# prashantpandeygit/solvingpapers

Measured on AMD Instinct MI355X. Metric: training tokens/sec, LLaMA3-8B-shape bf16, higher is better.
Workload: dtype bf16; 1 GPU; model=llama3_8b, global_batch=4, seq_len=8192, parallelism=dp1, micro_batch=1, grad_accum=4, params=8030261248

## Files before the change

### csrc/include/attn_params.h

```cpp
#pragma once
#include "attn_common.h"

#define SPA_DBG_BRH(b, r, R, h, H) (SPA_DBG_OK(b, p.B) & SPA_DBG_OK(r, R) & SPA_DBG_OK(h, H))

namespace spa {

struct AttnParams {
  const bf16* q; const bf16* k; const bf16* v; const bf16* o; const bf16* dout;
  bf16* out; bf16* dq; bf16* dk; bf16* dv;
  float* lse; const float* lse_in; float* delta; float* dqacc;
  int B, H, Hkv, Tq, Tk;
  long sqb, sqt, sqh, skb, skt, skh, svb, svt, svh, sob, sot, soh;
  long sdob, sdot, sdoh;
  long sdqb, sdqt, sdqh, sdkb, sdkt, sdkh, sdvb, sdvt, sdvh;
  float scale;
  float scale_log2;
  int causal_off;
  int hsplit;
  float* dkacc; float* dvacc;
  unsigned seed_lo, seed_hi, drop_thr;
  float drop_scale;
  const int64_t* seed_ptr;
  long long* stamp;
  int xcd;
  bf16* dsbuf;
  long ds_kvstride;
  int ds_nqt, ds_nkt;
  int ksplit;
  float* part;
  float* mlpart;
  int part_ld;
  int vhalf;
  float* rowk;
  int rowk_ld;
};

void launch_dkdv5(AttnParams& p, bool causal, hipStream_t st);
void launch_bwd_short(AttnParams& p, bool causal, hipStream_t st);

__device__ __forceinline__ long ds_index(int qt, int kt, int g, int G, int nkt, bool causal) {
  const int qb = qt >> 1, t = qt & 1;
  const long step = causal ? (long)qb * (qb + 1) + kt : (long)qb * nkt + kt;
  return (step * G + g) * 2 + t;
}
inline long ds_kv_elems(int nq64, int nkt, int G, bool causal) {
  return 1024L * 2 * G * (causal ? (long)nq64 * (nq64 + 1) : (long)nq64 * nkt);
}
__device__ __forceinline__ int ds_slot(int s, int h, int k) { return (k >> 2) * 16 + (2 * s + h) * 4 + (k & 3); }

template <int HD, int NDT = HD / 32>
__device__ __forceinline__ void store_kv_grad(const AttnParams& p, const f32x16 (&acc)[NDT], bool is_k,
                                              int b, int hk, int key, int split, int hh, int dt0 = 0) {
  if (key >= p.Tk) return;
  if (!(SPA_DBG_BRH(b, key, p.Tk, hk, p.Hkv) & SPA_DBG_OK(split, p.hsplit))) return;
  static_assert(NDT <= HD / 32, "store_kv_grad: more tiles than the head dim");
  constexpr int DT = NDT;
  if (p.hsplit == 1) {
    bf16* dst = (is_k ? p.dk + b * p.sdkb + (long)key * p.sdkt + hk * p.sdkh
                      : p.dv + b * p.sdvb + (long)key * p.sdvt + hk * p.sdvh) + 32 * dt0;
    const float sc = is_k ? p.scale : 1.f;
#pragma unroll
    for (int dt = 0; dt < DT; ++dt)
#pragma unroll
      for (int g = 0; g < 4; ++g) {
        bf16x4 w;
#pragma unroll
        for (int i = 0; i < 4; ++i) w[i] = (bf16)(acc[dt][4 * g + i] * sc);
        *reinterpret_cast<bf16x4*>(dst + 32 * dt + 8 * g + 4 * hh) = w;
      }
  } else {
    float* dst = (is_k ? p.dkacc : p.dvacc) +
                 ((((long)split * p.B + b) * p.Tk + key) * p.Hkv + hk) * HD + 32 * dt0;
#pragma unroll
    for (int dt = 0; dt < DT; ++dt)
#pragma unroll
      for (int g = 0; g < 4; ++g) {
        f32x4 w;
#pragma unroll
        for (int i = 0; i < 4; ++i) w[i] = acc[dt][4 * g + i];
        *reinterpret_cast<f32x4*>(dst + 32 * dt + 8 * g + 4 * hh) = w;
      }
  }
// ... 5 lines not shown
```

### csrc/include/spa_common.h

```cpp
#pragma once

#include <hip/hip_runtime.h>
#include <torch/library.h>
#include <ATen/ATen.h>
#include <ATen/hip/HIPContext.h>
#include <ATen/hip/impl/HIPGuardImplMasqueradingAsCUDA.h>
#include <cstdint>

#include "spa_debug.h"

namespace spa {

typedef __bf16 bf16;
typedef __bf16 bf16x8 __attribute__((ext_vector_type(8)));
typedef __bf16 bf16x4 __attribute__((ext_vector_type(4)));
typedef __bf16 bf16x2 __attribute__((ext_vector_type(2)));
typedef float f32x16 __attribute__((ext_vector_type(16)));
typedef float f32x4 __attribute__((ext_vector_type(4)));
typedef float f32x2 __attribute__((ext_vector_type(2)));
typedef unsigned short u16x8 __attribute__((ext_vector_type(8)));

constexpr int kWave = 64;

using DeviceGuard = c10::hip::HIPGuardMasqueradingAsCUDA;
// ... 30 lines not shown
}
template <int NT>
__device__ __forceinline__ float block_max(float v, float* red) {
  v = wave_max(v);
  const int w = threadIdx.x >> 6, l = threadIdx.x & 63;
  if (NT == 64) return v;
  __syncthreads();
  if (l == 0) red[w] = v;
  __syncthreads();
  float s = -INFINITY;
#pragma unroll
  for (int i = 0; i < NT / 64; ++i) s = fmaxf(s, red[i]);
  return s;
}

__device__ __forceinline__ void load8(const bf16* p, float (&f)[8]) {
  bf16x8 v = *reinterpret_cast<const bf16x8*>(p);
#pragma unroll
  for (int i = 0; i < 8; ++i) f[i] = (float)v[i];
}
__device__ __forceinline__ void store8(bf16* p, const float (&f)[8]) {
  bf16x8 v;
#pragma unroll
  for (int i = 0; i < 8; ++i) v[i] = (bf16)f[i];
  *reinterpret_cast<bf16x8*>(p) = v;
}
__device__ __forceinline__ void load8(const float* p, float (&f)[8]) {
  f32x4 a = *reinterpret_cast<const f32x4*>(p);
  f32x4 b = *reinterpret_cast<const f32x4*>(p + 4);
#pragma unroll
// ... 30 lines not shown
```

### csrc/kernels/attention.hip

```cpp
#include "attn_common.h"
#include "attn_params.h"

SPA_DEBUG_TU("attention.hip")

namespace spa {



__device__ __forceinline__ unsigned mix32(unsigned x) {
  x ^= x >> 16; x *= 0x7feb352dU; x ^= x >> 15; x *= 0x846ca68bU; x ^= x >> 16;
  return x;
}
__device__ __forceinline__ unsigned drop_base(const AttnParams& p, int b, int h) {
  unsigned lo = p.seed_lo, hi = p.seed_hi;
  if (p.seed_ptr) {
    const uint64_t sd = (uint64_t)*p.seed_ptr;
    lo = (unsigned)(sd & 0xffffffffu);
    hi = (unsigned)(sd >> 32);
  }
  return mix32(lo ^ mix32(hi + (unsigned)(b * p.H + h) * 0x9E3779B9U));
}
__device__ __forceinline__ bool drop_keep(unsigned base, int q, int key, unsigned thr) {
  return (mix32(base + (unsigned)q * 0x85EBCA6BU + (unsigned)key * 0xC2B2AE35U) >> 8) >= thr;
}
// ... 185 lines not shown
          for (int i = 0; i < 4; ++i) w[i] = o[dt][4 * g + i];
          *reinterpret_cast<f32x4*>(dst + 32 * dt + 8 * g + 4 * hh) = w;
        }
      if (hh == 0 && blockIdx.y == 0) {
        float2 ml;
        ml.x = m;
        ml.y = l;
        reinterpret_cast<float2*>(p.mlpart)[row] = ml;
      }
    }
    return;
  }
  const float inv = l > 0.f ? 1.f / l : 0.f;
  if (q < p.Tq && SPA_DBG_BRH(b, q, p.Tq, h, p.H)) {
    bf16* op = p.out + b * p.sob + (long)q * p.sot + h * p.soh + vcol;
#pragma unroll
    for (int dt = 0; dt < DT; ++dt)
#pragma unroll
      for (int g = 0; g < 4; ++g) {
        bf16x4 w;
#pragma unroll
        for (int i = 0; i < 4; ++i) w[i] = (bf16)(o[dt][4 * g + i] * inv);
        *reinterpret_cast<bf16x4*>(op + 32 * dt + 8 * g + 4 * hh) = w;
      }
    if (hh == 0 && p.lse)
      p.lse[((long)b * p.H + h) * p.Tq + q] = (l > 0.f) ? (m + __log2f(l)) * 0.69314718055994531f : INFINITY;
  }
}

template <bool CAUSAL>
__global__ __launch_bounds__(512) void attn_fwd256p_kernel(AttnParams p) {
  constexpr int HD = 256, BN = 32, BM = 128, KS = HD / 16, DH = 4, NT = 512;
  constexpr int TI = BN * HD;
  constexpr int PS = 4 * 2 * 64 * 8;
  __shared__ __attribute__((aligned(16))) bf16 smem[4 * TI + 2 * PS];
  __shared__ __attribute__((aligned(16))) float arow[2][4][64];
  const int tid = threadIdx.x, lane = tid & 63;
  const int wave = __builtin_amdgcn_readfirstlane(tid >> 6);
// ... 1073 lines not shown
        if (jj + 1 < nsteps) asm volatile("s_waitcnt vmcnt(6)" ::: "memory");
        else asm volatile("s_waitcnt vmcnt(0)" ::: "memory");
        asm volatile("s_waitcnt lgkmcnt(0)" ::: "memory");
        __builtin_amdgcn_s_barrier();
        if (jj + 2 < nsteps) issue(jj + 2, (r + 2) % 3);
        compute(jj, smem + r * SLOT);
      }
    }
  }
  if (!uvalid) return;
#pragma unroll
  for (int t = 0; t < 2; ++t) {
    const int q = qb * 64 + 32 * t + (lane & 31);
    if (q >= p.Tq || !SPA_DBG_BRH(b, q, p.Tq, h, p.H)) continue;
    bf16* op = p.dq + b * p.sdqb + (long)q * p.sdqt + h * p.sdqh;
#pragma unroll
    for (int dt = 0; dt < DT; ++dt)
#pragma unroll
      for (int g = 0; g < 4; ++g) {
        bf16x4 wv;
#pragma unroll
        for (int i = 0; i < 4; ++i) wv[i] = (bf16)(acc[t][dt][4 * g + i] * p.scale);
        *reinterpret_cast<bf16x4*>(op + 32 * dt + 8 * g + 4 * hh) = wv;
      }
  }
}

template <int HDK, bool CAUSAL, bool NT>
__global__ __launch_bounds__(256, 2) void attn_bwd_dq_ds256_kernel(AttnParams p) {
  static_assert(HDK == 256 || HDK == 192, "dq_ds256: q/k head dim 192 or 256");
  constexpr int HD = 256, DT = HDK / 32, KIMG = 32 * HD, WSLOT = 1024, SLOT = KIMG + 4 * WSLOT, NSLOT = 3;
  __shared__ __attribute__((aligned(16))) bf16 smem[NSLOT * SLOT];
  const int tid = threadIdx.x, lane = tid & 63;
  const int wave = __builtin_amdgcn_readfirstlane(tid >> 6);
  const int hh = lane >> 5;
  const int G = p.H / p.Hkv;
  const int nqt = cdiv(p.Tq, 32);
// ... 244 lines not shown
  constexpr int TPR = HD / 8;
  const long n = (long)p.B * p.Tq * p.H * TPR;
  for (long i = blockIdx.x * 256L + threadIdx.x; i < n; i += (long)gridDim.x * 256) {
    const int t = i % TPR;
    const long row = i / TPR;
    const long h = row % p.H, q = (row / p.H) % p.Tq, b = row / ((long)p.H * p.Tq);
    float a[8];
    load8(p.dqacc + row * HD + 8 * t, a);
#pragma unroll
    for (int k = 0; k < 8; ++k) a[k] *= p.scale;
    if (SPA_DBG_BRH(b, q, p.Tq, h, p.H)) store8(p.dq + b * p.sdqb + q * p.sdqt + h * p.sdqh + 8 * t, a);
  }
}


static void check_qkv(const at::Tensor& t, const char* n) {
  TORCH_CHECK(t.is_cuda() && t.scalar_type() == at::kBFloat16, n, " must be a bf16 HIP tensor");
  TORCH_CHECK(t.dim() == 4, n, " must be [B, T, H, hd]");
  TORCH_CHECK(t.stride(3) == 1, n, " must be contiguous in hd");
  TORCH_CHECK(((uintptr_t)t.data_ptr() % 16) == 0 && t.stride(1) % 8 == 0 && t.stride(2) % 8 == 0 &&
                  t.stride(0) % 8 == 0,
              n, ": rows must be 16-byte aligned");
}

template <int HDK, int HDV> constexpr int fwd_waves() {
  return (HDK <= 192 && HDV <= 192) || (HDK == 256 && HDV == 128) ? 8 : 4;
}
template <int HDK, int HDV> constexpr int dq_waves() { return (HDK <= 128 && HDV <= 128) ? 8 : 4; }

#define HDKV_SWITCH(HK, HV, ...)                                                                   \
// ... 26 lines not shown
  p.seed_hi = (unsigned)(((uint64_t)seed >> 32) & 0xffffffffu);
  p.drop_thr = (unsigned)std::llround(dropout_p * 16777216.0);
  p.drop_scale = (float)(1.0 / (1.0 - dropout_p));
}

static int attn_ksplit(long blocks, int ntk) {
  const char* e = getenv("SPA_ATTN_KSPLIT");
  if (e) return std::max(1, std::min(atoi(e), std::max(1, ntk)));
  int ks = 1;
  while (blocks * ks < 512 && ks < 8 && ntk / (2 * ks) >= 4) ks *= 2;
  return ks;
}

std::vector<at::Tensor> attn_fwd(const at::Tensor& q, const at::Tensor& k, const at::Tensor& v, double scale,
                                 bool causal, double dropout_p, int64_t seed,
                                 const c10::optional<at::Tensor>& seed_t) {
  check_qkv(q, "q"); check_qkv(k, "k"); check_qkv(v, "v");
  const int B = q.size(0), Tq = q.size(1), H = q.size(2), HDK = q.size(3), HDV = v.size(3);
  const int Tk = k.size(1), Hkv = k.size(2);
  TORCH_CHECK(k.size(0) == B && v.size(0) == B && v.size(1) == Tk && v.size(2) == Hkv && k.size(3) == HDK,
              "attn: shape mismatch");
  TORCH_CHECK(H % Hkv == 0, "attn: H must be a multiple of Hkv");
  const bool drop = dropout_p > 0.0;
  TORCH_CHECK(!drop || HDK == HDV, "attn: dropout needs equal q/k and v head dims");
  DeviceGuard g(q.device());
  auto out = at::empty({B, Tq, H, HDV}, q.options());
  auto lse = at::empty({B, H, Tq}, q.options().dtype(at::kFloat));
  AttnParams p{};
  p.q = (const bf16*)q.data_ptr(); p.k = (const bf16*)k.data_ptr(); p.v = (const bf16*)v.data_ptr();
  p.out = (bf16*)out.data_ptr(); p.lse = lse.data_ptr<float>();
  p.B = B; p.H = H; p.Hkv = Hkv; p.Tq = Tq; p.Tk = Tk;
  fill_strides(p, q, k, v);
  fill_dropout(p, dropout_p, seed, seed_t);
  p.sob = out.stride(0); p.sot = out.stride(1); p.soh = out.stride(2);
  p.scale = (float)scale; p.scale_log2 = (float)(scale * 1.4426950408889634);
  p.causal_off = Tk - Tq;
  p.hsplit = 1;
  p.ksplit = 1;
  p.xcd = xcd_order(B, Hkv);
  if (B * Tq * H == 0) return {out, lse};
  auto st = stream();
  const char* f2e = getenv("SPA_ATTN_FWD256");
  const bool pshare = !(f2e && atoi(f2e) == 0) && HDK == 256 && HDV == 256 && !drop;
  const char* sve = getenv("SPA_ATTN_SPLITV");
  const bool splitv = !pshare && !(sve && atoi(sve) == 0) && HDK == 256 && HDV == 256 && !drop;
  const int nw = splitv || pshare ? 8 : (HDK <= 192 && HDV <= 192) || (HDK == 256 && HDV == 128) ? 8 : 4;
  const int blocks = cdiv(Tq, pshare ? 128 : 32 * nw) * H * B * (splitv ? 2 : 1);
  const int ntk = cdiv(Tk, (HDK >= 256 || HDV >= 256) ? 32 : 64);
  p.ksplit = attn_ksplit(blocks, ntk);
  at::Tensor part;
  if (p.ksplit > 1) {
    const long rows = (long)B * H * Tq;
    part = at::empty({(long)p.ksplit * rows * (HDV + 2)}, q.options().dtype(at::kFloat));
    p.part = part.data_ptr<float>();
    p.part_ld = HDV;
    p.mlpart = p.part + (long)p.ksplit * rows * HDV;
  }
  const int gx = blocks / (splitv ? 2 : 1) * p.ksplit;
  if (pshare) {
    if (causal) attn_fwd256p_kernel<true><<<gx, 512, 0, st>>>(p);
    else attn_fwd256p_kernel<false><<<gx, 512, 0, st>>>(p);
  } else if (splitv) {
    p.vhalf = 128;
    if (causal) attn_fwd_kernel<256, 128, 8, true, false><<<dim3(gx, 2), 512, 0, st>>>(p);
    else attn_fwd_kernel<256, 128, 8, false, false><<<dim3(gx, 2), 512, 0, st>>>(p);
  } else {
    HDKV_SWITCH(HDK, HDV, {
      constexpr int NW = fwd_waves<HDK_, HDV_>();
      constexpr bool SQ = HDK_ == HDV_;
      if (drop) {
        if constexpr (SQ) {
          if (causal) attn_fwd_kernel<HDK_, HDV_, NW, true, true><<<gx, NW * 64, 0, st>>>(p);
          else attn_fwd_kernel<HDK_, HDV_, NW, false, true><<<gx, NW * 64, 0, st>>>(p);
        }
      } else {
        if (causal) attn_fwd_kernel<HDK_, HDV_, NW, true, false><<<gx, NW * 64, 0, st>>>(p);
        else attn_fwd_kernel<HDK_, HDV_, NW, false, false><<<gx, NW * 64, 0, st>>>(p);
      }
    });
  }
  if (p.ksplit > 1) {
    const long n = (long)B * H * Tq * (HDV / 8);
    HDKV_SWITCH(HDK, HDV, { attn_fwd_merge_kernel<HDV_><<<(int)cdiv(n, 256L), 256, 0, st>>>(p); });
  }
  SPA_LAUNCH_CHECK();
  return {out, lse};
}

template <int HDK, int HDV, bool DROP>
static void launch_bwd(AttnParams& p, bool causal, bool fused, int dkdv_mode, int nkv, hipStream_t st,
                       const at::TensorOptions& bf16_opts) {
  constexpr int NW = dq_waves<HDK, HDV>();
  constexpr int MT = (HDK <= 128 && HDV <= 128) ? 2 : 1;
  constexpr bool PAIRED_OK = HDK == HDV && HDK <= 128 && !DROP;
  const int g2 = nkv * p.hsplit;
  if constexpr (HDK == HDV && HDK <= 128 && !DROP) {
    if (fused) {
      const long rows = (long)p.B * p.Tq * p.H;
      attn_delta_kernel<HDK><<<(int)cdiv(rows, 256 / (HDK / 8)), 256, 0, st>>>(p);
      if (causal) attn_bwd_dkdv_kernel<HDK, HDV, true, MT, true, false><<<g2, 256, 0, st>>>(p);
// ... 7 lines not shown
    const char* de = getenv("SPA_ATTN_DQ_DS");
    const bool want = !(de && atoi(de) == 0);
    const long kv_bytes = 2 * ds_kv_elems(cdiv(p.Tq, 64), cdiv(p.Tk, 32), p.H / p.Hkv, causal);
    if (want && p.hsplit == 1 && p.Tk > 0 && dkdv_mode == 0 && (!causal || p.causal_off == 0) &&
        kv_bytes < 0x7fffffffL) {
      const long rows = (long)p.B * p.Tq * p.H;
      const char* v5e = getenv("SPA_ATTN_DKDV5");
      const bool v5 = !(v5e && atoi(v5e) == 0);
      if (!v5) attn_delta_kernel<HDK><<<(int)cdiv(rows, 256 / (HDK / 8)), 256, 0, st>>>(p);
      p.ds_nqt = cdiv(p.Tq, 32);
      p.ds_nkt = cdiv(p.Tk, 32);
      p.ds_kvstride = ds_kv_elems(cdiv(p.Tq, 64), p.ds_nkt, p.H / p.Hkv, causal);
      at::Tensor dsb = at::empty({(long)p.B * p.Hkv * p.ds_kvstride}, bf16_opts);
      p.dsbuf = (bf16*)dsb.data_ptr();
      at::Tensor rowk;
      if (v5) {
        p.rowk_ld = cdiv(p.Tq, 64) * 64;
        rowk = at::empty({(long)p.B * p.H * 2 * p.rowk_ld}, bf16_opts.dtype(at::kFloat));
        p.rowk = rowk.data_ptr<float>();
        launch_dkdv5(p, causal, st);
      } else if (causal) attn_bwd_dkdv3_kernel<HDK, HDV, true, true><<<nkv, 512, 0, st>>>(p);
      else attn_bwd_dkdv3_kernel<HDK, HDV, false, true><<<nkv, 512, 0, st>>>(p);
      const int G = p.H / p.Hkv;
      const int wg = cdiv(cdiv(p.Tq, 64) * G, 4) * p.B * p.Hkv;
      const char* ne = getenv("SPA_ATTN_DS_NT");
      const bool nt = !(ne && atoi(ne) == 0);
      if (nt) {
        if (causal) attn_bwd_dq_ds_kernel<HDK, true, true><<<wg, 256, 0, st>>>(p);
        else attn_bwd_dq_ds_kernel<HDK, false, true><<<wg, 256, 0, st>>>(p);
      } else {
// ... 102 lines not shown
    const long rows = (long)p.B * p.Tk * p.Hkv;
    attn_kv_reduce_kernel<HDK><<<(int)std::min<long>((rows * (HDK / 8) + 255) / 256, 65536), 256, 0, st>>>(p, 1);
    attn_kv_reduce_kernel<HDV><<<(int)std::min<long>((rows * (HDV / 8) + 255) / 256, 65536), 256, 0, st>>>(p, 0);
  }
}

static at::Tensor& last_stamps() {
  static at::Tensor t;
  return t;
}
at::Tensor attn_bwd_stamps() { return last_stamps().defined() ? last_stamps().view({-1, 8}).clone() : at::Tensor(); }

void attn_bwd(const at::Tensor& dout, const at::Tensor& q, const at::Tensor& k, const at::Tensor& v,
              const at::Tensor& out, const at::Tensor& lse, const at::Tensor& dq, const at::Tensor& dk,
              const at::Tensor& dv, double scale, bool causal, double dropout_p, int64_t seed,
              const c10::optional<at::Tensor>& seed_t) {
  check_qkv(dout, "dout"); check_qkv(q, "q"); check_qkv(k, "k"); check_qkv(v, "v"); check_qkv(out, "out");
  check_qkv(dq, "dq"); check_qkv(dk, "dk"); check_qkv(dv, "dv");
  const int B = q.size(0), Tq = q.size(1), H = q.size(2), HDK = q.size(3), HDV = v.size(3);
  const int Tk = k.size(1), Hkv = k.size(2);
  TORCH_CHECK(lse.is_contiguous() && lse.numel() == (int64_t)B * H * Tq);
  TORCH_CHECK(dq.sizes() == q.sizes() && dk.sizes() == k.sizes() && dv.sizes() == v.sizes());
  TORCH_CHECK(dout.sizes() == out.sizes() && out.size(3) == HDV && out.size(2) == H && out.size(1) == Tq);
  const bool drop = dropout_p > 0.0;
  TORCH_CHECK(!drop || HDK == HDV, "attn: dropout needs equal q/k and v head dims");
  DeviceGuard g(q.device());
  auto delta = at::empty({B, H, Tq}, q.options().dtype(at::kFloat));
  AttnParams p{};
  p.q = (const bf16*)q.data_ptr(); p.k = (const bf16*)k.data_ptr(); p.v = (const bf16*)v.data_ptr();
  p.o = (const bf16*)out.data_ptr(); p.dout = (const bf16*)dout.data_ptr();
  p.dq = (bf16*)dq.data_ptr(); p.dk = (bf16*)dk.data_ptr(); p.dv = (bf16*)dv.data_ptr();
  p.lse_in = lse.data_ptr<float>(); p.delta = delta.data_ptr<float>();
  p.B = B; p.H = H; p.Hkv = Hkv; p.Tq = Tq; p.Tk = Tk;
  fill_strides(p, q, k, v);
  fill_dropout(p, dropout_p, seed, seed_t);
  p.sob = out.stride(0); p.sot = out.stride(1); p.soh = out.stride(2);
  p.sdob = dout.stride(0); p.sdot = dout.stride(1); p.sdoh = dout.stride(2);
  p.sdqb = dq.stride(0); p.sdqt = dq.stride(1); p.sdqh = dq.stride(2);
  p.sdkb = dk.stride(0); p.sdkt = dk.stride(1); p.sdkh = dk.stride(2);
  p.sdvb = dv.stride(0); p.sdvt = dv.stride(1); p.sdvh = dv.stride(2);
  p.scale = (float)scale; p.scale_log2 = (float)(scale * 1.4426950408889634);
  p.causal_off = Tk - Tq;
  p.xcd = xcd_order(B, Hkv);
  p.ksplit = 1;
  if (B * H == 0) return;
  auto st = stream();
  if (Tq == 0) { dk.zero_(); dv.zero_(); return; }
  static const bool want_fused = getenv("SPA_ATTN_BWD_FUSED") && atoi(getenv("SPA_ATTN_BWD_FUSED")) != 0;
  const bool fused = want_fused && Tk > 0 && HDK <= 128 && HDK == HDV && !drop;
  const char* sse = getenv("SPA_ATTN_SHORT");
  const bool want_short = !(sse && atoi(sse) == 0);
  if (want_short && !fused && !drop && HDK == 64 && HDV == 64 && H == Hkv && Tq <= 256 && Tk <= 256) {
    launch_bwd_short(p, causal, st);
    SPA_LAUNCH_CHECK();
    return;
  }
  at::Tensor dqacc;
  if (fused) {
    dqacc = at::zeros({B, Tq, H, HDK}, q.options().dtype(at::kFloat));
    p.dqacc = dqacc.data_ptr<float>();
  }
  const int dkdv_mode = getenv("SPA_ATTN_DKDV") ? atoi(getenv("SPA_ATTN_DKDV")) : 0;
  const int G = H / Hkv;
  const int nkv = cdiv(Tk, 128) * Hkv * B;
  int hsplit = 1;
  const char* kbe = getenv("SPA_ATTN_KVBLOCKS");
  const int kvblocks = kbe ? std::max(1, atoi(kbe)) : 512;
  if (!fused)
    while (nkv * hsplit < kvblocks && hsplit < G) {
// ... 16 lines not shown
  }
  at::Tensor kvacc;
  if (hsplit > 1) {
    kvacc = at::empty({(long)hsplit * B * Tk * Hkv * (HDK + HDV)}, q.options().dtype(at::kFloat));
    p.dkacc = kvacc.data_ptr<float>();
    p.dvacc = p.dkacc + (long)hsplit * B * Tk * Hkv * HDK;
  }
  HDKV_SWITCH(HDK, HDV, {
    if (drop) {
      if constexpr (HDK_ == HDV_) launch_bwd<HDK_, HDV_, true>(p, causal, false, dkdv_mode, nkv, st, q.options());
    } else {
      launch_bwd<HDK_, HDV_, false>(p, causal, fused, dkdv_mode, nkv, st, q.options());
    }
  });
  SPA_LAUNCH_CHECK();
}

}

TORCH_LIBRARY_FRAGMENT(spa, m) {
  m.def("attn_fwd(Tensor q, Tensor k, Tensor v, float scale, bool causal, float dropout_p=0.0, int seed=0, "
        "Tensor? seed_t=None) -> Tensor[]");
  m.def("attn_bwd(Tensor dout, Tensor q, Tensor k, Tensor v, Tensor out, Tensor lse, Tensor(a!) dq, Tensor(b!) dk, "
        "Tensor(c!) dv, float scale, bool causal, float dropout_p=0.0, int seed=0, Tensor? seed_t=None) -> ()");
  m.def("attn_bwd_stamps() -> Tensor", &spa::attn_bwd_stamps);
}
TORCH_LIBRARY_IMPL(spa, CUDA, m) {
  m.impl("attn_fwd", &spa::attn_fwd);
  m.impl("attn_bwd", &spa::attn_bwd);
}
```

### csrc/kernels/attention_dkdv5.hip

```cpp
#include "attn_common.h"
#include "attn_params.h"

SPA_DEBUG_TU("attention_dkdv5.hip")

namespace spa {

__device__ __forceinline__ void dma4_asm(__amdgpu_buffer_rsrc_t rs, unsigned voff, unsigned lds) {
  unsigned keep;
  asm volatile("s_mov_b32 %0, m0\n\ts_mov_b32 m0, %3\n\ts_nop 0\n\tbuffer_load_dword %1, %2, 0 offen lds\n\ts_mov_b32 m0, %0"
               : "=&s"(keep) : "v"(voff), "s"(rs), "s"(lds) : "memory");
}

template <int HD>
__global__ __launch_bounds__(256) void attn_rowk_kernel(AttnParams p) {
  constexpr int TPR = HD / 8, RPB = 256 / TPR;
  const int Tqp = p.rowk_ld;
  const long row = (long)blockIdx.x * RPB + threadIdx.x / TPR;
  const int t = threadIdx.x % TPR;
  const long nrows = (long)p.B * Tqp * p.H;
  float acc = 0.f;
  long b = 0, q = 0, h = 0;
  if (row < nrows) {
    h = row % p.H;
    q = (row / p.H) % Tqp;
// ... 276 lines not shown
  };
  if (total == 0) {
  } else if (role == 0) {
    for (int k = 0; k <= total; k += 3) {
      interval(k, IC<0>{}, IC<0>{});
      interval(k + 1, IC<1>{}, IC<0>{});
      interval(k + 2, IC<2>{}, IC<0>{});
    }
  } else {
    for (int k = 0; k <= total; k += 3) {
      interval(k, IC<0>{}, IC<1>{});
      interval(k + 1, IC<1>{}, IC<1>{});
      interval(k + 2, IC<2>{}, IC<1>{});
    }
  }
  store_kv_grad<HD>(p, acc, role == 1, b, hk, key, 0, hh);
#if SPA_DKDV5_STAMP
  D5_TICK(4);
  if (p.stamp != nullptr && lane < 8) {
    long long v = 0;
#pragma unroll
    for (int i = 0; i < 5; ++i) v = lane == i ? seg[i] : v;
    v = lane == 5 ? (long long)(total + 1) : lane == 6 ? ts_ - t_start : v;
    p.stamp[((long)blockIdx.x * 8 + wave) * 8 + lane] = v;
  }
#endif
}

void launch_dkdv5(AttnParams& p, bool causal, hipStream_t st) {
  const long rows = (long)p.B * p.rowk_ld * p.H;
  attn_rowk_kernel<128><<<(int)cdiv(rows, 256 / 16), 256, 0, st>>>(p);
// ... 7 lines not shown
```

### csrc/kernels/layout.hip

```cpp
#include "spa_common.h"

namespace spa {

#ifndef SPA_TRANSPOSE_TS
#define SPA_TRANSPOSE_TS 64
#endif
#ifndef SPA_TRANSPOSE_DIAG
#define SPA_TRANSPOSE_DIAG 0
#endif
template <typename T>
__global__ __launch_bounds__(256) void transpose_kernel(const T* __restrict__ x, T* __restrict__ y, int R, int C,
                                                        long ldx, long ldy, long bsx, long bsy) {
  x += blockIdx.z * bsx;
  y += blockIdx.z * bsy;
  constexpr int TS = SPA_TRANSPOSE_TS, PAD = 16 / sizeof(T), LD = TS + PAD, VE = 16 / sizeof(T);
  __shared__ __attribute__((aligned(16))) T tile[TS * LD];
#if SPA_TRANSPOSE_DIAG
  const int bx = (blockIdx.x + blockIdx.y) % gridDim.x;
  const int r0 = blockIdx.y * TS, c0 = bx * TS;
#else
  const int r0 = blockIdx.y * TS, c0 = blockIdx.x * TS;
#endif
  constexpr int CPR = TS / VE;
  constexpr int NCH = TS * CPR;
// ... 36 lines not shown
  if (R == 0 || C == 0 || Bt == 0) return y;
  dim3 grid(cdiv(C, SPA_TRANSPOSE_TS), cdiv(R, SPA_TRANSPOSE_TS), Bt);
  const long ld = x.stride(-2), bsx = batched ? x.stride(0) : 0, bsy = (long)R * C;
  if (x.scalar_type() == at::kBFloat16)
    transpose_kernel<bf16><<<grid, 256, 0, stream()>>>((const bf16*)x.data_ptr(), (bf16*)y.data_ptr(), R, C, ld, R,
                                                       bsx, bsy);
  else if (x.scalar_type() == at::kFloat)
    transpose_kernel<float><<<grid, 256, 0, stream()>>>(x.data_ptr<float>(), y.data_ptr<float>(), R, C, ld, R, bsx,
                                                        bsy);
  else
    TORCH_CHECK(false, "transpose2d: bf16/fp32");
  SPA_LAUNCH_CHECK();
  return y;
}

__global__ __launch_bounds__(256) void stream_copy_wg_kernel(const uint4* __restrict__ src, uint4* __restrict__ dst,
                                                             long n, int reps) {
  for (int r = 0; r < reps; ++r)
    for (long i = blockIdx.x * 256L + threadIdx.x; i < n; i += (long)gridDim.x * 256) dst[i] = src[i];
}

void stream_copy_wg(const at::Tensor& src, at::Tensor& dst, int64_t nwg, int64_t reps) {
  SPA_CHECK_CUDA(src);
  TORCH_CHECK(src.is_contiguous() && dst.is_contiguous() && src.nbytes() == dst.nbytes() && src.nbytes() % 16 == 0,
              "stream_copy_wg: contiguous, equal sizes, 16-byte multiple");
  TORCH_CHECK(nwg > 0 && nwg <= 65536 && reps >= 0, "stream_copy_wg: nwg in [1, 65536], reps >= 0");
  DeviceGuard g(src.device());
  const long n = (long)(src.nbytes() / 16);
  if (n == 0 || reps == 0) return;
  stream_copy_wg_kernel<<<(int)nwg, 256, 0, stream()>>>((const uint4*)src.data_ptr(), (uint4*)dst.data_ptr(), n,
// ... 15 lines not shown
```

### csrc/kernels/rope.hip

```cpp
#include "spa_common.h"
#include <type_traits>

namespace spa {

template <typename DT, int MODE>
__global__ __launch_bounds__(256) void rope_kernel(DT* __restrict__ x, const float* __restrict__ cosT,
                                                   const float* __restrict__ sinT, const int* __restrict__ pos,
                                                   long sb, long st, long sh, int B, int T, int nrot, int hd,
                                                   int pos_off, float sign) {
  const int vpr = hd / 8;
  const long total = (long)B * T * nrot * vpr;
  for (long i = blockIdx.x * 256L + threadIdx.x; i < total; i += (long)gridDim.x * 256) {
    const int v = i % vpr;
    long r = i / vpr;
    const int hh = r % nrot;
    r /= nrot;
    const int t = r % T;
    const int b = r / T;
    const int ps = pos ? pos[b * T + t] : t + pos_off;
    DT* p = x + b * sb + t * st + hh * sh;
    const float* c = cosT + (long)ps * (hd / 2);
    const float* s = sinT + (long)ps * (hd / 2);
    if constexpr (MODE == 0 || MODE == 2) {
      float a[8];
      load8(p + v * 8, a);
      const f32x4 cv = *reinterpret_cast<const f32x4*>(c + v * 4);
      const f32x4 sv = *reinterpret_cast<const f32x4*>(s + v * 4);
#pragma unroll
      for (int k = 0; k < 4; ++k) {
        const float x0 = a[2 * k], x1 = a[2 * k + 1];
        const float cs = cv[k];
        if constexpr (MODE == 0) {
          const float sn = sign * sv[k];
          a[2 * k] = x0 * cs - x1 * sn;
          a[2 * k + 1] = x0 * sn + x1 * cs;
        } else if (sign > 0.f) {
          a[2 * k] = cs * (x0 + x1);
          a[2 * k + 1] = sv[k] * (x1 - x0);
        } else {
          a[2 * k] = cs * x0 - sv[k] * x1;
          a[2 * k + 1] = cs * x0 + sv[k] * x1;
        }
      }
      store8(p + v * 8, a);
    } else {
      if (v >= vpr / 2) continue;
      float a[8], bq[8];
      load8(p + v * 8, a);
      load8(p + hd / 2 + v * 8, bq);
      float cv[8], sv[8];
// ... 167 lines not shown
```

### solvingpapers_amd/models/llama3.py

```python
from __future__ import annotations

import math
from dataclasses import dataclass, field, replace
from typing import List, Optional

import torch
import torch.nn as nn

from ..infer.cache import KVCache
from ..infer.graph import DecodeState
from ..infer.sampling import sample
from ..ops import _ext, attention_packed, embedding, linear, linear_cross_entropy, rms_norm, rope_packed_
from ..ops.linear import swiglu_mlp
from ..ops.attention import decode_attention
from ..ops.rope import RopeCache, apply_rope
from ..utils.grad import mark_ready


@dataclass
class LlamaConfig:
    vocab_size: int = 50257
    dim: int = 256
    n_layers: int = 2
    n_heads: int = 4
    n_kv_heads: int = 2
    ffn_hidden: int = 1024
    max_seq_len: int = 128
    norm_eps: float = 1e-6
    rope_theta: float = 10000.0
# ... 61 lines not shown
            x4 = qkv.view(B, T, H + 2 * KV, hd)
            cos, sin = RopeCache.get(pos.max_len, hd, c.rope_theta, qkv.device, c.ref_freqs)
            kc, vc = kv_cache
            _ext.ops().rope_kv_write_(x4, cos, sin, pos.positions, pos.index, kc, vc, H, KV, 0)
            o = decode_attention(x4[:, :, :H], kc, vc, causal=True, kv_len=pos.kv_len)
            return linear(o.reshape(B, T, H * hd), self.wo)
        if kv_cache is None and self.cp_group is not None:
            import torch.distributed as dist
            from ..parallel.context_parallel import context_parallel_attention
            H, KV = c.n_heads, c.n_kv_heads
            off = dist.get_rank(self.cp_group) * T
            qkv = rope_packed_(qkv, H + KV, c.rope_theta, off, head_dim=hd, ref_freqs=c.ref_freqs)
            x4 = qkv.view(B, T, H + 2 * KV, hd)
            o = context_parallel_attention(x4[:, :, :H], x4[:, :, H:H + KV], x4[:, :, H + KV:], self.cp_group)
        elif kv_cache is None:
            qkv = rope_packed_(qkv, c.n_heads + c.n_kv_heads, c.rope_theta, 0, head_dim=hd, ref_freqs=c.ref_freqs)
            o = attention_packed(qkv, c.n_heads, c.n_kv_heads, causal=True, head_dim=hd)
        else:
            qkv = qkv.view(B, T, c.n_heads + 2 * c.n_kv_heads, hd)
            q = apply_rope(qkv[:, :, :c.n_heads], c.rope_theta, pos, ref_freqs=c.ref_freqs)
            k = apply_rope(qkv[:, :, c.n_heads:c.n_heads + c.n_kv_heads], c.rope_theta, pos, ref_freqs=c.ref_freqs)
            v = qkv[:, :, c.n_heads + c.n_kv_heads:]
            kc, vc = kv_cache
            kc[:, pos:pos + T] = k
            vc[:, pos:pos + T] = v
            o = decode_attention(q, kc[:, :pos + T], vc[:, :pos + T], causal=True)
        return linear(o.reshape(B, T, c.n_heads * hd), self.wo)

    def forward(self, res, delta, kv_cache=None, pos=0):
        c = self.c
        if res is None:
            n1 = rms_norm(delta, self.attention_norm, c.norm_eps)
# ... 152 lines not shown
```

### solvingpapers_amd/ops/attention.py

```python
from __future__ import annotations

import math

import os

import torch

from . import _ext, reference

FLASH_PAIRS = ((64, 64), (128, 128), (256, 256), (192, 128))
FLASH_HD = (64, 128, 256)


def _pair_for(dqk, dv):
    best = None
    for a, b in FLASH_PAIRS:
        if a >= dqk and b >= dv and (best is None or a + b < best[0] + best[1]):
            best = (a, b)
    return best


def _flash_ok(q):
    return q.is_cuda and q.dtype == torch.bfloat16 and (q.dim() == 3 or q.shape[-1] in FLASH_HD)

# ... 65 lines not shown
        ctx.dropout_p, ctx.seed = dropout_p, seed
        return torch.ops.aten._unsafe_view(out, (B, T, H * hd))

    @staticmethod
    def backward(ctx, dout):
        qkv, out, lse = ctx.saved_tensors
        H, Hkv, hd = ctx.H, ctx.Hkv, ctx.hd
        B, T = qkv.shape[0], qkv.shape[1]
        dqkv = torch.empty_like(qkv)
        x4 = qkv.view(B, T, H + 2 * Hkv, hd)
        d4 = dqkv.view(B, T, H + 2 * Hkv, hd)
        _ext.ops().attn_bwd(dout.contiguous().view(B, T, H, hd), x4[:, :, :H], x4[:, :, H:H + Hkv],
                            x4[:, :, H + Hkv:], out, lse, d4[:, :, :H], d4[:, :, H:H + Hkv], d4[:, :, H + Hkv:],
                            ctx.scale, ctx.causal, ctx.dropout_p, *_seed_args(ctx.seed))
        return dqkv, None, None, None, None, None, None, None


FLASH_F32_HD = (16, 32, 64, 128, 256)


class _FlashF32Fn(torch.autograd.Function):

    @staticmethod
    def forward(ctx, q, k, v, causal, scale, dropout_p, seed):
        si, st = _seed_args(seed)
        out, lse = _ext.ops().attn_f32_fwd(q, k, v, scale, causal, dropout_p, si, st)
        ctx.save_for_backward(q, k, v, out, lse)
        ctx.causal, ctx.scale, ctx.dropout_p, ctx.seed = causal, scale, dropout_p, seed
        return out

# ... 252 lines not shown
```

### solvingpapers_amd/ops/layout.py

```python
from __future__ import annotations

import os

import torch

from . import _ext

WGRAD_NT = os.environ.get("SPA_WGRAD_NT", "1") != "0"
WGRAD_NT_MIN_TOKENS = 2048
WGRAD_NT_MIN_WIDTH = 2048
WGRAD8 = os.environ.get("SPA_WGRAD8", "1") != "0"
WGRAD8_MIN_TOKENS = 4096


def transpose2d(x: torch.Tensor) -> torch.Tensor:
    if x.is_cuda and x.dtype in (torch.bfloat16, torch.float32):
        return _ext.ops().transpose2d(x)
    return x.transpose(-1, -2).contiguous()


def wgrad_nt_ok(dy2: torch.Tensor, x2: torch.Tensor) -> bool:
    return (WGRAD_NT and dy2.is_cuda and dy2.dtype == torch.bfloat16 and x2.dtype == torch.bfloat16
            and dy2.shape[0] >= WGRAD_NT_MIN_TOKENS and dy2.shape[0] % 8 == 0
            and dy2.shape[1] % 8 == 0 and x2.shape[1] % 8 == 0
            and dy2.stride(1) == 1 and x2.stride(1) == 1 and dy2.stride(0) % 8 == 0 and x2.stride(0) % 8 == 0)


def wgrad_operand(dy2: torch.Tensor, x2: torch.Tensor):
    if wgrad_nt_ok(dy2, x2) and min(dy2.shape[1], x2.shape[1]) >= WGRAD_NT_MIN_WIDTH and x2.shape[1] <= dy2.shape[1]:
        return transpose2d(x2)
    return None


def wgrad8_ok(dy2: torch.Tensor, x2: torch.Tensor, out=None) -> bool:
    return (WGRAD8 and dy2.is_cuda and dy2.dtype == torch.bfloat16 and x2.dtype == torch.bfloat16
            and dy2.dim() == 2 and x2.dim() == 2 and dy2.shape[0] >= WGRAD8_MIN_TOKENS
            and min(dy2.shape[1], x2.shape[1]) < WGRAD_NT_MIN_WIDTH
            and dy2.shape[1] % 8 == 0 and x2.shape[1] % 8 == 0 and dy2.stride(1) == 1 and x2.stride(1) == 1
            and dy2.stride(0) % 8 == 0 and x2.stride(0) % 8 == 0
            and dy2.data_ptr() % 16 == 0 and x2.data_ptr() % 16 == 0
            and (out is None or (out.is_contiguous() and out.dtype in (torch.bfloat16, torch.float32))))


def wgrad(dy2: torch.Tensor, x2: torch.Tensor, out=None, accumulate=False, x2t=None, dyt=None):
    if dyt is None and wgrad8_ok(dy2, x2, out):
        return _ext.ops().wgrad8(dy2, x2, out, accumulate, 0)
# ... 47 lines not shown
```

### solvingpapers_amd/ops/linear.py

```python
from __future__ import annotations

import os
import weakref

import torch

from ..utils.grad import commit
from . import _ext
from .layout import bias_grad, wgrad

GEMV = os.environ.get("SPA_GEMV", "1") != "0"
GEMV_MAX_ROWS = 4

DGRAD_WT = os.environ.get("SPA_DGRAD_WT", "1") != "0"
DGRAD_WT_MIN_NUMEL = int(os.environ.get("SPA_DGRAD_WT_MIN", str(1 << 18)))
_WT_CACHE: dict = {}


def invalidate_weight_caches():
    from .moe import bump_weight_epoch
    bump_weight_epoch()


def transposed_weight(w: torch.Tensor):
# ... 51 lines not shown
    @staticmethod
    def backward(ctx, dy):
        (x,) = ctx.saved_tensors
        w, b = ctx.w, ctx.b
        dy2 = dy.reshape(-1, dy.shape[-1])
        x2 = x.reshape(-1, x.shape[-1])
        dx = dgrad(dy2, w).view(x.shape) if ctx.needs_input_grad[0] else None
        gw = gb = None
        if ctx.needs_input_grad[1]:
            def _w(out, acc):
                return wgrad(dy2, x2, out, acc)
            gw = commit(w, _w)
        if b is not None and ctx.needs_input_grad[2]:
            gb = _commit_bias(b, bias_grad(dy2))
        return dx, gw, gb


class _LinearActFn(torch.autograd.Function):

    @staticmethod
    def forward(ctx, x, w, b, kind, alpha):
        x2 = x.reshape(-1, x.shape[-1])
        u = torch.addmm(b, x2, w.t())
        y = _ext.ops().act_fwd(u, kind, alpha)
        ctx.save_for_backward(x, u)
        ctx.w, ctx.b, ctx.kind, ctx.alpha = w, b, kind, alpha
        return torch.ops.aten._unsafe_view(y, (*x.shape[:-1], w.shape[0]))

    @staticmethod
    def backward(ctx, dy):
# ... 324 lines not shown
```

Before: 21940 tokens/s.

## Fuse RoPE backward into attention bwd stores and emit transposed attention output

Adds a packed rope+attention autograd function that applies the inverse RoPE rotation to dq and dk directly in the attention backward store epilogues, replacing separate rope passes over the gradients. The attention forward can also write a transposed copy of its output, which the wo projection's weight-gradient GEMM uses in place of a separate transpose. In exchange the backward kernels gain extra cos/sin table loads and register pressure, and the strided transposed stores in the forward epilogue are uncoalesced.

```diff
diff --git a/csrc/include/attn_params.h b/csrc/include/attn_params.h
--- a/csrc/include/attn_params.h
+++ b/csrc/include/attn_params.h
@@ -33,10 +33,39 @@
   int vhalf;
   float* rowk;
   int rowk_ld;
+  bf16* out_t;
+  long ot_ld;
+  const float* rope_cos; const float* rope_sin;
+  int rope_pos_off;
+  int rope_fuse;
 };
 
 void launch_dkdv5(AttnParams& p, bool causal, hipStream_t st);
 void launch_bwd_short(AttnParams& p, bool causal, hipStream_t st);
+
+__device__ __forceinline__ void rope_bwd4(bf16x4& w, const f32x2 cv, const f32x2 sv) {
+#pragma unroll
+  for (int k = 0; k < 2; ++k) {
+    float x0 = (float)w[2 * k], x1 = (float)w[2 * k + 1];
+    rope_pair(x0, x1, cv[k], -sv[k]);
+    w[2 * k] = (bf16)x0;
+    w[2 * k + 1] = (bf16)x1;
+  }
+}
+template <int DT>
+struct RopeRow {
+  f32x2 c[DT][4], s[DT][4];
+  __device__ __forceinline__ void load(const AttnParams& p, int pos, int half_dim, int hh, int dt0 = 0) {
+    const long ro = (long)pos * half_dim + 16 * dt0 + 2 * hh;
+#pragma unroll
+    for (int dt = 0; dt < DT; ++dt)
+#pragma unroll
+      for (int g = 0; g < 4; ++g) {
+        c[dt][g] = *reinterpret_cast<const f32x2*>(p.rope_cos + ro + 16 * dt + 4 * g);
+        s[dt][g] = *reinterpret_cast<const f32x2*>(p.rope_sin + ro + 16 * dt + 4 * g);
+      }
+  }
+};
 
 __device__ __forceinline__ long ds_index(int qt, int kt, int g, int G, int nkt, bool causal) {
   const int qb = qt >> 1, t = qt & 1;
@@ -48,7 +77,7 @@
 }
 __device__ __forceinline__ int ds_slot(int s, int h, int k) { return (k >> 2) * 16 + (2 * s + h) * 4 + (k & 3); }
 
-template <int HD, int NDT = HD / 32>
+template <int HD, int NDT = HD / 32, bool ROPE = false>
 __device__ __forceinline__ void store_kv_grad(const AttnParams& p, const f32x16 (&acc)[NDT], bool is_k,
                                               int b, int hk, int key, int split, int hh, int dt0 = 0) {
   if (key >= p.Tk) return;
@@ -59,6 +88,12 @@
     bf16* dst = (is_k ? p.dk + b * p.sdkb + (long)key * p.sdkt + hk * p.sdkh
                       : p.dv + b * p.sdvb + (long)key * p.sdvt + hk * p.sdvh) + 32 * dt0;
     const float sc = is_k ? p.scale : 1.f;
+    bool rot = false;
+    RopeRow<ROPE ? DT : 1> rr;
+    if constexpr (ROPE) {
+      rot = is_k && p.rope_fuse;
+      if (rot) rr.load(p, key + p.rope_pos_off, HD / 2, hh, dt0);
+    }
 #pragma unroll
     for (int dt = 0; dt < DT; ++dt)
 #pragma unroll
@@ -66,6 +101,9 @@
         bf16x4 w;
 #pragma unroll
         for (int i = 0; i < 4; ++i) w[i] = (bf16)(acc[dt][4 * g + i] * sc);
+        if constexpr (ROPE) {
+          if (rot) rope_bwd4(w, rr.c[dt][g], rr.s[dt][g]);
+        }
         *reinterpret_cast<bf16x4*>(dst + 32 * dt + 8 * g + 4 * hh) = w;
       }
   } else {
diff --git a/csrc/include/spa_common.h b/csrc/include/spa_common.h
--- a/csrc/include/spa_common.h
+++ b/csrc/include/spa_common.h
@@ -68,6 +68,14 @@
   return s;
 }
 
+__device__ __forceinline__ void rope_pair(float& x0, float& x1, float cs, float sn) {
+#pragma clang fp contract(off)
+  const float a = x0, b = x1;
+  const float t0 = b * sn, t1 = a * sn;
+  x0 = __builtin_fmaf(a, cs, -t0);
+  x1 = __builtin_fmaf(b, cs, t1);
+}
+
 __device__ __forceinline__ void load8(const bf16* p, float (&f)[8]) {
   bf16x8 v = *reinterpret_cast<const bf16x8*>(p);
 #pragma unroll
diff --git a/csrc/kernels/attention.hip b/csrc/kernels/attention.hip
--- a/csrc/kernels/attention.hip
+++ b/csrc/kernels/attention.hip
@@ -223,6 +223,7 @@
   const float inv = l > 0.f ? 1.f / l : 0.f;
   if (q < p.Tq && SPA_DBG_BRH(b, q, p.Tq, h, p.H)) {
     bf16* op = p.out + b * p.sob + (long)q * p.sot + h * p.soh + vcol;
+    bf16* tp = p.out_t ? p.out_t + ((long)h * HDV + 4 * hh) * p.ot_ld + (long)b * p.Tq + q : nullptr;
 #pragma unroll
     for (int dt = 0; dt < DT; ++dt)
 #pragma unroll
@@ -231,6 +232,10 @@
 #pragma unroll
         for (int i = 0; i < 4; ++i) w[i] = (bf16)(o[dt][4 * g + i] * inv);
         *reinterpret_cast<bf16x4*>(op + 32 * dt + 8 * g + 4 * hh) = w;
+        if (tp) {
+#pragma unroll
+          for (int i = 0; i < 4; ++i) tp[(32 * dt + 8 * g + i) * p.ot_ld] = w[i];
+        }
       }
     if (hh == 0 && p.lse)
       p.lse[((long)b * p.H + h) * p.Tq + q] = (l > 0.f) ? (m + __log2f(l)) * 0.69314718055994531f : INFINITY;
@@ -1334,6 +1339,8 @@
     const int q = qb * 64 + 32 * t + (lane & 31);
     if (q >= p.Tq || !SPA_DBG_BRH(b, q, p.Tq, h, p.H)) continue;
     bf16* op = p.dq + b * p.sdqb + (long)q * p.sdqt + h * p.sdqh;
+    RopeRow<DT> rr;
+    if (p.rope_fuse) rr.load(p, q + p.rope_pos_off, HD / 2, hh);
 #pragma unroll
     for (int dt = 0; dt < DT; ++dt)
 #pragma unroll
@@ -1341,6 +1348,7 @@
         bf16x4 wv;
 #pragma unroll
         for (int i = 0; i < 4; ++i) wv[i] = (bf16)(acc[t][dt][4 * g + i] * p.scale);
+        if (p.rope_fuse) rope_bwd4(wv, rr.c[dt][g], rr.s[dt][g]);
         *reinterpret_cast<bf16x4*>(op + 32 * dt + 8 * g + 4 * hh) = wv;
       }
   }
@@ -1615,6 +1623,10 @@
 }
 
 
+void transpose2d_into(const at::Tensor& x, const at::Tensor& y);
+void rope_(const at::Tensor& x, const at::Tensor& cos, const at::Tensor& sin, const c10::optional<at::Tensor>& pos,
+           int64_t nrot, int64_t pos_off, int64_t mode, bool inverse);
+
 static void check_qkv(const at::Tensor& t, const char* n) {
   TORCH_CHECK(t.is_cuda() && t.scalar_type() == at::kBFloat16, n, " must be a bf16 HIP tensor");
   TORCH_CHECK(t.dim() == 4, n, " must be [B, T, H, hd]");
@@ -1671,7 +1683,8 @@
 
 std::vector<at::Tensor> attn_fwd(const at::Tensor& q, const at::Tensor& k, const at::Tensor& v, double scale,
                                  bool causal, double dropout_p, int64_t seed,
-                                 const c10::optional<at::Tensor>& seed_t) {
+                                 const c10::optional<at::Tensor>& seed_t,
+                                 const c10::optional<at::Tensor>& out_t) {
   check_qkv(q, "q"); check_qkv(k, "k"); check_qkv(v, "v");
   const int B = q.size(0), Tq = q.size(1), H = q.size(2), HDK = q.size(3), HDV = v.size(3);
   const int Tk = k.size(1), Hkv = k.size(2);
@@ -1695,6 +1708,11 @@
   p.hsplit = 1;
   p.ksplit = 1;
   p.xcd = xcd_order(B, Hkv);
+  if (out_t) {
+    TORCH_CHECK(out_t->is_cuda() && out_t->scalar_type() == at::kBFloat16 && out_t->is_contiguous() &&
+                    out_t->dim() == 2 && out_t->size(0) == (int64_t)H * HDV && out_t->size(1) == (int64_t)B * Tq,
+                "attn: out_t must be a contiguous bf16 [H*dv, B*Tq] tensor");
+  }
   if (B * Tq * H == 0) return {out, lse};
   auto st = stream();
   const char* f2e = getenv("SPA_ATTN_FWD256");
@@ -1713,6 +1731,11 @@
     p.part_ld = HDV;
     p.mlpart = p.part + (long)p.ksplit * rows * HDV;
   }
+  const bool ot_fused = out_t && !pshare && !splitv && p.ksplit == 1;
+  if (ot_fused) {
+    p.out_t = (bf16*)out_t->data_ptr();
+    p.ot_ld = (long)B * Tq;
+  }
   const int gx = blocks / (splitv ? 2 : 1) * p.ksplit;
   if (pshare) {
     if (causal) attn_fwd256p_kernel<true><<<gx, 512, 0, st>>>(p);
@@ -1741,6 +1764,7 @@
     HDKV_SWITCH(HDK, HDV, { attn_fwd_merge_kernel<HDV_><<<(int)cdiv(n, 256L), 256, 0, st>>>(p); });
   }
   SPA_LAUNCH_CHECK();
+  if (out_t && !ot_fused) transpose2d_into(out.view({(int64_t)B * Tq, (int64_t)H * HDV}), *out_t);
   return {out, lse};
 }
 
@@ -1778,6 +1802,8 @@
       at::Tensor dsb = at::empty({(long)p.B * p.Hkv * p.ds_kvstride}, bf16_opts);
       p.dsbuf = (bf16*)dsb.data_ptr();
       at::Tensor rowk;
+      const char* rbe = getenv("SPA_ATTN_ROPE_BWD");
+      p.rope_fuse = (v5 && p.rope_cos && !(rbe && atoi(rbe) == 0)) ? 1 : 0;
       if (v5) {
         p.rowk_ld = cdiv(p.Tq, 64) * 64;
         rowk = at::empty({(long)p.B * p.H * 2 * p.rowk_ld}, bf16_opts.dtype(at::kFloat));
@@ -1910,7 +1936,8 @@
 void attn_bwd(const at::Tensor& dout, const at::Tensor& q, const at::Tensor& k, const at::Tensor& v,
               const at::Tensor& out, const at::Tensor& lse, const at::Tensor& dq, const at::Tensor& dk,
               const at::Tensor& dv, double scale, bool causal, double dropout_p, int64_t seed,
-              const c10::optional<at::Tensor>& seed_t) {
+              const c10::optional<at::Tensor>& seed_t, const c10::optional<at::Tensor>& rope_cos,
+              const c10::optional<at::Tensor>& rope_sin, int64_t rope_pos_off) {
   check_qkv(dout, "dout"); check_qkv(q, "q"); check_qkv(k, "k"); check_qkv(v, "v"); check_qkv(out, "out");
   check_qkv(dq, "dq"); check_qkv(dk, "dk"); check_qkv(dv, "dv");
   const int B = q.size(0), Tq = q.size(1), H = q.size(2), HDK = q.size(3), HDV = v.size(3);
@@ -1939,6 +1966,29 @@
   p.causal_off = Tk - Tq;
   p.xcd = xcd_order(B, Hkv);
   p.ksplit = 1;
+  const bool rope = rope_cos.has_value();
+  if (rope) {
+    TORCH_CHECK(rope_sin.has_value(), "attn_bwd: rope_cos and rope_sin come together");
+    for (auto* t : {&*rope_cos, &*rope_sin})
+      TORCH_CHECK(t->is_cuda() && t->scalar_type() == at::kFloat && t->is_contiguous() && t->dim() == 2 &&
+                      t->size(1) == HDK / 2, "attn_bwd: rope tables must be contiguous fp32 [Tmax, dk/2]");
+    TORCH_CHECK(rope_pos_off >= 0 && rope_pos_off + std::max(Tq, Tk) <= rope_cos->size(0) &&
+                    rope_sin->size(0) == rope_cos->size(0), "attn_bwd: rope table too short");
+    p.rope_cos = rope_cos->data_ptr<float>();
+    p.rope_sin = rope_sin->data_ptr<float>();
+    p.rope_pos_off = (int)rope_pos_off;
+  }
+  auto rope_back = [&]() {
+    if (!rope || p.rope_fuse) return;
+    if (dk.data_ptr() == (void*)((bf16*)dq.data_ptr() + (int64_t)H * dq.stride(2)) && dk.strides() == dq.strides() &&
+        Tq == Tk && dq.stride(2) == HDK) {
+      rope_(dq.as_strided({B, Tq, H + Hkv, HDK}, dq.strides()), *rope_cos, *rope_sin, c10::nullopt, H + Hkv,
+            rope_pos_off, 0, true);
+    } else {
+      rope_(dq, *rope_cos, *rope_sin, c10::nullopt, H, rope_pos_off, 0, true);
+      rope_(dk, *rope_cos, *rope_sin, c10::nullopt, Hkv, rope_pos_off, 0, true);
+    }
+  };
   if (B * H == 0) return;
   auto st = stream();
   if (Tq == 0) { dk.zero_(); dv.zero_(); return; }
@@ -1949,6 +1999,7 @@
   if (want_short && !fused && !drop && HDK == 64 && HDV == 64 && H == Hkv && Tq <= 256 && Tk <= 256) {
     launch_bwd_short(p, causal, st);
     SPA_LAUNCH_CHECK();
+    rope_back();
     return;
   }
   at::Tensor dqacc;
@@ -1995,15 +2046,17 @@
     }
   });
   SPA_LAUNCH_CHECK();
+  rope_back();
 }
 
 }
 
 TORCH_LIBRARY_FRAGMENT(spa, m) {
   m.def("attn_fwd(Tensor q, Tensor k, Tensor v, float scale, bool causal, float dropout_p=0.0, int seed=0, "
-        "Tensor? seed_t=None) -> Tensor[]");
+        "Tensor? seed_t=None, Tensor(a!)? out_t=None) -> Tensor[]");
   m.def("attn_bwd(Tensor dout, Tensor q, Tensor k, Tensor v, Tensor out, Tensor lse, Tensor(a!) dq, Tensor(b!) dk, "
-        "Tensor(c!) dv, float scale, bool causal, float dropout_p=0.0, int seed=0, Tensor? seed_t=None) -> ()");
+        "Tensor(c!) dv, float scale, bool causal, float dropout_p=0.0, int seed=0, Tensor? seed_t=None, "
+        "Tensor? rope_cos=None, Tensor? rope_sin=None, int rope_pos_off=0) -> ()");
   m.def("attn_bwd_stamps() -> Tensor", &spa::attn_bwd_stamps);
 }
 TORCH_LIBRARY_IMPL(spa, CUDA, m) {
diff --git a/csrc/kernels/attention_dkdv5.hip b/csrc/kernels/attention_dkdv5.hip
--- a/csrc/kernels/attention_dkdv5.hip
+++ b/csrc/kernels/attention_dkdv5.hip
@@ -314,7 +314,7 @@
       interval(k + 2, IC<2>{}, IC<1>{});
     }
   }
-  store_kv_grad<HD>(p, acc, role == 1, b, hk, key, 0, hh);
+  store_kv_grad<HD, HD / 32, true>(p, acc, role == 1, b, hk, key, 0, hh);
 #if SPA_DKDV5_STAMP
   D5_TICK(4);
   if (p.stamp != nullptr && lane < 8) {
diff --git a/csrc/kernels/layout.hip b/csrc/kernels/layout.hip
--- a/csrc/kernels/layout.hip
+++ b/csrc/kernels/layout.hip
@@ -74,6 +74,22 @@
   return y;
 }
 
+void transpose2d_into(const at::Tensor& x, const at::Tensor& y) {
+  SPA_CHECK_CUDA(x);
+  TORCH_CHECK(x.dim() == 2 && x.stride(1) == 1 && x.scalar_type() == at::kBFloat16, "transpose2d_into: bf16 [R, C]");
+  const int R = x.size(0), C = x.size(1);
+  TORCH_CHECK(y.is_cuda() && y.scalar_type() == at::kBFloat16 && y.is_contiguous() && y.dim() == 2 &&
+                  y.size(0) == C && y.size(1) == R, "transpose2d_into: y must be contiguous bf16 [C, R]");
+  TORCH_CHECK(R % 8 == 0 && C % 8 == 0 && x.stride(0) % 8 == 0 && (uintptr_t)x.data_ptr() % 16 == 0 &&
+                  (uintptr_t)y.data_ptr() % 16 == 0, "transpose2d_into: rows/cols must be 16-byte multiples");
+  DeviceGuard g(x.device());
+  if (R == 0 || C == 0) return;
+  dim3 grid(cdiv(C, SPA_TRANSPOSE_TS), cdiv(R, SPA_TRANSPOSE_TS), 1);
+  transpose_kernel<bf16><<<grid, 256, 0, stream()>>>((const bf16*)x.data_ptr(), (bf16*)y.data_ptr(), R, C,
+                                                     x.stride(0), R, 0, 0);
+  SPA_LAUNCH_CHECK();
+}
+
 __global__ __launch_bounds__(256) void stream_copy_wg_kernel(const uint4* __restrict__ src, uint4* __restrict__ dst,
                                                              long n, int reps) {
   for (int r = 0; r < reps; ++r)
diff --git a/csrc/kernels/rope.hip b/csrc/kernels/rope.hip
--- a/csrc/kernels/rope.hip
+++ b/csrc/kernels/rope.hip
@@ -31,9 +31,7 @@
         const float x0 = a[2 * k], x1 = a[2 * k + 1];
         const float cs = cv[k];
         if constexpr (MODE == 0) {
-          const float sn = sign * sv[k];
-          a[2 * k] = x0 * cs - x1 * sn;
-          a[2 * k + 1] = x0 * sn + x1 * cs;
+          rope_pair(a[2 * k], a[2 * k + 1], cs, sign * sv[k]);
         } else if (sign > 0.f) {
           a[2 * k] = cs * (x0 + x1);
           a[2 * k + 1] = sv[k] * (x1 - x0);
diff --git a/solvingpapers_amd/models/llama3.py b/solvingpapers_amd/models/llama3.py
--- a/solvingpapers_amd/models/llama3.py
+++ b/solvingpapers_amd/models/llama3.py
@@ -11,8 +11,9 @@
 from ..infer.graph import DecodeState
 from ..infer.sampling import sample
 from ..ops import _ext, attention_packed, embedding, linear, linear_cross_entropy, rms_norm, rope_packed_
-from ..ops.linear import swiglu_mlp
-from ..ops.attention import decode_attention
+from ..ops.linear import linear_xt, swiglu_mlp
+from ..ops.attention import decode_attention, rope_attention_packed
+from ..ops.layout import wgrad_takes_x2t
 from ..ops.rope import RopeCache, apply_rope
 from ..utils.grad import mark_ready
 
@@ -104,8 +105,11 @@
             x4 = qkv.view(B, T, H + 2 * KV, hd)
             o = context_parallel_attention(x4[:, :, :H], x4[:, :, H:H + KV], x4[:, :, H + KV:], self.cp_group)
         elif kv_cache is None:
-            qkv = rope_packed_(qkv, c.n_heads + c.n_kv_heads, c.rope_theta, 0, head_dim=hd, ref_freqs=c.ref_freqs)
-            o = attention_packed(qkv, c.n_heads, c.n_kv_heads, causal=True, head_dim=hd)
+            want_t = (torch.is_grad_enabled() and self.wo.requires_grad and self.wo.dtype == torch.bfloat16
+                      and wgrad_takes_x2t(B * T, self.wo.shape[0], c.n_heads * hd))
+            o, o_t = rope_attention_packed(qkv, c.n_heads, c.n_kv_heads, hd, c.rope_theta, 0, causal=True,
+                                           ref_freqs=c.ref_freqs, want_t=want_t)
+            return linear_xt(o, o_t, self.wo)
         else:
             qkv = qkv.view(B, T, c.n_heads + 2 * c.n_kv_heads, hd)
             q = apply_rope(qkv[:, :, :c.n_heads], c.rope_theta, pos, ref_freqs=c.ref_freqs)
diff --git a/solvingpapers_amd/ops/attention.py b/solvingpapers_amd/ops/attention.py
--- a/solvingpapers_amd/ops/attention.py
+++ b/solvingpapers_amd/ops/attention.py
@@ -103,6 +103,52 @@
                             x4[:, :, H + Hkv:], out, lse, d4[:, :, :H], d4[:, :, H:H + Hkv], d4[:, :, H + Hkv:],
                             ctx.scale, ctx.causal, ctx.dropout_p, *_seed_args(ctx.seed))
         return dqkv, None, None, None, None, None, None, None
+
+
+class _RopePackedFn(torch.autograd.Function):
+
+    @staticmethod
+    def forward(ctx, qkv, H, Hkv, hd, causal, scale, cos, sin, pos_off, want_t):
+        ops = _ext.ops()
+        B, T = qkv.shape[0], qkv.shape[1]
+        x4 = qkv.view(B, T, H + 2 * Hkv, hd)
+        ops.rope_(x4, cos, sin, None, H + Hkv, pos_off, 0, False)
+        o_t = torch.empty(H * hd, B * T, device=qkv.device, dtype=qkv.dtype) if want_t else None
+        out, lse = ops.attn_fwd(x4[:, :, :H], x4[:, :, H:H + Hkv], x4[:, :, H + Hkv:], scale, causal, 0.0, 0, None,
+                                o_t)
+        ctx.save_for_backward(qkv, out, lse)
+        ctx.args = (H, Hkv, hd, causal, scale, cos, sin, pos_off)
+        o = torch.ops.aten._unsafe_view(out, (B, T, H * hd))
+        if o_t is not None:
+            ctx.mark_non_differentiable(o_t)
+        return o, o_t
+
+    @staticmethod
+    def backward(ctx, dout, _dot=None):
+        qkv, out, lse = ctx.saved_tensors
+        H, Hkv, hd, causal, scale, cos, sin, pos_off = ctx.args
+        B, T = qkv.shape[0], qkv.shape[1]
+        dqkv = torch.empty_like(qkv)
+        x4 = qkv.view(B, T, H + 2 * Hkv, hd)
+        d4 = dqkv.view(B, T, H + 2 * Hkv, hd)
+        _ext.ops().attn_bwd(dout.contiguous().view(B, T, H, hd), x4[:, :, :H], x4[:, :, H:H + Hkv],
+                            x4[:, :, H + Hkv:], out, lse, d4[:, :, :H], d4[:, :, H:H + Hkv], d4[:, :, H + Hkv:],
+                            scale, causal, 0.0, 0, None, cos, sin, pos_off)
+        return (dqkv,) + (None,) * 9
+
+
+def rope_attention_packed(qkv, H, Hkv, head_dim, theta=10000.0, pos_off=0, causal=True, scale=None,
+                          ref_freqs=False, want_t=False):
+    from .rope import RopeCache, rope_packed_
+    hd = head_dim
+    B, T = qkv.shape[0], qkv.shape[1]
+    scale = float(scale) if scale is not None else 1.0 / math.sqrt(hd)
+    if qkv.is_cuda and qkv.dtype == torch.bfloat16 and hd in FLASH_HD and qkv.is_contiguous():
+        cos, sin = RopeCache.get(pos_off + T, hd, theta, qkv.device, ref_freqs)
+        want_t = bool(want_t) and os.environ.get("SPA_ATTN_OT", "1") != "0"
+        return _RopePackedFn.apply(qkv, H, Hkv, hd, causal, scale, cos, sin, int(pos_off), want_t)
+    qkv = rope_packed_(qkv, H + Hkv, theta, pos_off, head_dim=hd, ref_freqs=ref_freqs)
+    return attention_packed(qkv, H, Hkv, causal=causal, scale=scale, head_dim=hd), None
 
 
 FLASH_F32_HD = (16, 32, 64, 128, 256)
diff --git a/solvingpapers_amd/ops/layout.py b/solvingpapers_amd/ops/layout.py
--- a/solvingpapers_amd/ops/layout.py
+++ b/solvingpapers_amd/ops/layout.py
@@ -30,6 +30,11 @@
     if wgrad_nt_ok(dy2, x2) and min(dy2.shape[1], x2.shape[1]) >= WGRAD_NT_MIN_WIDTH and x2.shape[1] <= dy2.shape[1]:
         return transpose2d(x2)
     return None
+
+
+def wgrad_takes_x2t(tokens: int, N: int, K: int) -> bool:
+    return (WGRAD_NT and tokens >= WGRAD_NT_MIN_TOKENS and tokens % 8 == 0 and N % 8 == 0 and K % 8 == 0
+            and min(N, K) >= WGRAD_NT_MIN_WIDTH and K <= N)
 
 
 def wgrad8_ok(dy2: torch.Tensor, x2: torch.Tensor, out=None) -> bool:
diff --git a/solvingpapers_amd/ops/linear.py b/solvingpapers_amd/ops/linear.py
--- a/solvingpapers_amd/ops/linear.py
+++ b/solvingpapers_amd/ops/linear.py
@@ -89,6 +89,34 @@
         if b is not None and ctx.needs_input_grad[2]:
             gb = _commit_bias(b, bias_grad(dy2))
         return dx, gw, gb
+
+
+class _LinearXtFn(torch.autograd.Function):
+
+    @staticmethod
+    def forward(ctx, x, x_t, w):
+        ctx.w = w
+        ctx.save_for_backward(x, x_t)
+        y = torch.mm(x.reshape(-1, x.shape[-1]), w.t())
+        return torch.ops.aten._unsafe_view(y, (*x.shape[:-1], w.shape[0]))
+
+    @staticmethod
+    def backward(ctx, dy):
+        x, x_t = ctx.saved_tensors
+        w = ctx.w
+        dy2 = dy.reshape(-1, dy.shape[-1])
+        x2 = x.reshape(-1, x.shape[-1])
+        dx = dgrad(dy2, w).view(x.shape) if ctx.needs_input_grad[0] else None
+        gw = None
+        if ctx.needs_input_grad[2]:
+            gw = commit(w, lambda out, acc: wgrad(dy2, x2, out, acc, x2t=x_t))
+        return dx, None, gw
+
+
+def linear_xt(x, x_t, w):
+    if x_t is None:
+        return linear(x, w)
+    return _LinearXtFn.apply(x, x_t, w)
 
 
 class _LinearActFn(torch.autograd.Function):
```

Result: no change. 21960 tokens/s, median of 6 (+0.1%).
